# kouyt5/lightning-asr

Hardware: AMD Instinct MI355X
Metric: audio-seconds/sec training (asr13x1, bs=32, 10 s clips) (higher is better)
Workload: dtype bf16; 1 GPU; asr13x1 QuartzNet-CTC train step, bs=32/GPU, 10 s synthetic 16 kHz clips, labels.txt vocab (C=28), HIP mel+conv+CTC+NovoGrad, random-init weights; global_batch=32, n_class=28, parallelism=dp1, feature_prefetch=True, hip_graph=True, staged_backward=False

## Files before the change

lightning_asr_amd/csrc/fused.h:

```cpp
#pragma once
#include "common.h"

namespace lasr {

int dwconv_fwd_bn(const void* y, const float* coef, const void* y2, const float* coef2, int act, const float* w, void* out, void* u,
                  int64_t B, int64_t T, int64_t C, int k, void* stream);

static constexpr int kDwTapRow = 160;
struct DwTapJobs {
  int n; int blk0[17]; const float* w[16]; uint32_t* out[16]; int C[16]; int k[16];
};
__device__ __forceinline__ uint32_t dw_tap_entry(const float* __restrict__ w, int C, int k, int e) {
  const int flip = e / (C * kDwTapRow), r = e - flip * (C * kDwTapRow);
  const int c = r / kDwTapRow, idx = r - c * kDwTapRow;
  const int i0 = idx < kDwTapRow / 2 ? 2 * idx : 2 * (idx - kDwTapRow / 2) + 1;
  const int j0 = i0 - 24, j1 = i0 - 23;
  const float* wc = w + (size_t)c * k;
  const int q0 = min(max(j0, 0), k - 1), q1 = min(max(j1, 0), k - 1);
  const float a0 = wc[flip ? k - 1 - q0 : q0], a1 = wc[flip ? k - 1 - q1 : q1];
  const uint32_t m0 = (j0 >= 0 && j0 < k) ? 0xffffffffu : 0u, m1 = (j1 >= 0 && j1 < k) ? 0xffffffffu : 0u;
  return (uint32_t)f32_to_bf16(__uint_as_float(__float_as_uint(a0) & m0)) | ((uint32_t)f32_to_bf16(__uint_as_float(__float_as_uint(a1) & m1)) << 16);
}
struct DwTapCtx { int n; const float* w[16]; const uint32_t* t[16]; int C[16]; };
void dw_taps_set_ctx(const DwTapCtx* ctx);
const uint32_t* dw_taps_for(const float* w, int flip, int64_t C);
bool dw_taps_enabled();

int mask_lengths_step_cast(const float* pct, int64_t B, int64_t T_, int32_t* lens, uint64_t* step_counter, const float* in, void* out,
                           int64_t n, const DwTapJobs* jobs, void* stream);
int head_tail(const float* gl, int64_t rows, int64_t C, void* gl_bf16, int64_t ld_out, float* bias_grad, void* workspace,
              size_t workspace_bytes, const float* nll, int64_t n_nll, float scale, float* loss, void* stream);

int bn_se_act_fwd(const void* y, const float* coef, const void* y2, const float* coef2, const float* sums, const float* W1, const float* W2,
                  void* out, float* pooled, float* hidden, float* scale, int dtype, int64_t B, int64_t T_, int64_t C, int act, void* stream);

bool log_softmax_split_on(int64_t C);
int log_softmax_split(const float* partials, int split, const float* bias, float* logits, float* logp, int32_t* argmax, int64_t N, int64_t C,
                      void* stream);

}
```

lightning_asr_amd/csrc/model.hip:

```cpp
#include "common.h"
#include "mel.h"
#include "fused.h"
#include "gemm.h"
#include "lstm_body.h"
#include "se_seqsum.h"
#include <string>
#include <vector>
#include <math.h>

extern "C" size_t lasr_bn_bwd_workspace_bytes(int64_t B, int64_t T, int64_t C);
extern "C" size_t lasr_gemm_workspace_bytes(int64_t M, int64_t N, int split_k, int want_stats);
extern "C" size_t lasr_dwconv_wgrad_workspace_bytes(int64_t B, int64_t Tout, int64_t C, int k);
extern "C" int lasr_log_softmax_bwd(const float*, const float*, float*, int64_t, int64_t, void*);
extern "C" int lasr_cast_f32_to_bf16(const float*, void*, int64_t, void*);
extern "C" int lasr_colsum_f32(const float* x, float* out, int64_t rows, int64_t C, void* workspace, size_t workspace_bytes, void* stream);
extern "C" size_t lasr_colsum_workspace_bytes(int64_t rows, int64_t C);
extern "C" int lasr_scale_sum_f32(const float* x, int64_t n, float scale, float* out, void* stream);
extern "C" int lasr_seqsum(const void* x, int dtype, int64_t B, int64_t T, int64_t C, float* sums, void* stream);
extern "C" int lasr_se_fwd(const float* sums, const float* coef, const float* W1, const float* W2, int64_t B, int64_t T, int64_t C,
                           float* pooled, float* hidden, float* scale, void* stream);
extern "C" size_t lasr_se_bwd_workspace_bytes(int64_t B, int64_t C);
extern "C" int lasr_se_bwd(const void* dout, const void* y, const float* coef, const void* y2, const float* coef2, const float* scale,
                           const float* hidden, const float* pooled, const float* W1, const float* W2, int dtype, int64_t B, int64_t T,
                           int64_t C, int act, float* seg, float* dW1, float* dW2, void* workspace, size_t workspace_bytes, void* stream);
// ... 60 lines not shown
  size_t o_wgp = 0, wgp_bytes = 0, o_dwp = 0, dwp_bytes = 0, o_dy = 0, o_dy2 = 0;
  size_t o_taps = 0;
};

struct LstmRef { int64_t w_ih[2] = {-1, -1}, w_hh[2] = {-1, -1}, b_ih[2] = {-1, -1}, b_hh[2] = {-1, -1}; };

struct Plan {
  int64_t B = 0, T_in = 0, T = 0, S_max = 0;
  size_t total = 0;
  size_t o_lens = 0, o_logits = 0, o_glogits = 0, o_nll = 0, o_scratch = 0, o_g[2] = {0, 0}, o_d1 = 0, o_d2 = 0, o_du = 0, o_dxr = 0;
  size_t o_sums = 0, o_sums2 = 0, o_ctc = 0, o_wbf16 = 0;
  size_t o_cat = 0, o_gx[2] = {0, 0}, o_lstm_saved = 0, o_dg[2] = {0, 0};
  size_t o_dgb[2] = {0, 0}, o_lstm_part = 0, o_lstm_bpart = 0, o_lstm_wgp = 0, lstm_wgp_bytes = 0;
  size_t scratch_bytes = 0, ctc_bytes = 0;
  size_t o_rowstat = 0, o_lean = 0, lean_bytes = 0;
};

}

using namespace lasr;

struct lasr_model {
  lasr_model_config cfg;
  std::vector<TensorInfo> tensors;
  std::vector<Unit> units;
  int64_t n_param = 0, n_buffer = 0;
  int64_t w_dec = -1, b_dec = -1;
  LstmRef lstm;
  Plan plan;
  bool planned = false;
  float drop_p = 0.f;
  uint64_t drop_seed = 0;
  uint64_t* drop_step = nullptr;
  const float* tail_nll = nullptr; float* tail_loss = nullptr;
  bool lean_active = false;
  int lean_tiles = 0;
  int bwd_cur = 0;
  bool taps_valid = false;
  int bwd_next = -1;
  struct Prefetch {
    bool armed = false;
    WaveSrc src; const int32_t* sample_lens; const int32_t* aug;
    int64_t B, L; int normalize; void* out_btf; int dtype; int32_t* frames_out; float* pct_out; void* ws; size_t ws_bytes;
  } prefetch;

  int64_t add_tensor(const std::string& name, std::initializer_list<int64_t> shape, int kind) {
    TensorInfo t;
    t.name = name;
    t.kind = kind;
    t.ndim = (int)shape.size();
    int i = 0;
    for (int64_t s : shape) { t.shape[i++] = s; t.numel *= s; }
    if (kind == 0) { t.offset = n_param; n_param += t.numel; }
    else if (kind == 1) { t.offset = n_buffer; n_buffer += t.numel; }
// ... 172 lines not shown
  p.o_g[1] = take(cur, (size_t)N * cmax * es);
  p.o_d1 = take(cur, (size_t)N * std::max<int64_t>(cmax, (C + 7) / 8 * 8) * es);
  p.o_d2 = take(cur, (size_t)N * cmax * es);
  p.o_du = take(cur, (size_t)N * cmax * es);
  p.o_dxr = take(cur, (size_t)N * cmax * es);
  p.o_sums = take(cur, 2 * cmax * sizeof(float));
  p.o_sums2 = take(cur, 2 * cmax * sizeof(float));
  p.ctc_bytes = lasr_ctc_workspace_bytes(B, p.T, S_max);
  p.o_ctc = take(cur, p.ctc_bytes);
  if (lean_capable(m)) {
    p.o_rowstat = take(cur, lasr_gemm_rowstat_bytes(N, C));
    p.lean_bytes = lasr_ctc_lean_workspace_bytes(B, p.T, C, S_max);
    p.o_lean = take(cur, p.lean_bytes);
  }
  if (m->cfg.dtype == LASR_BF16) p.o_wbf16 = take(cur, (size_t)m->n_param * sizeof(bf16_t));
  p.total = cur;
  m->planned = true;
}

extern "C" int lasr_model_create(const lasr_model_config* cfg, lasr_model_t** out) {
  LASR_CHECK_ARG(cfg && out, "lasr_model_create: null pointer");
  LASR_CHECK_ARG(cfg->variant >= 0 && cfg->variant <= 2 && cfg->n_class >= 2 && cfg->in_c > 0 && cfg->in_c % 4 == 0,
                 "lasr_model_create: bad config (variant=%d n_class=%d in_c=%d)", cfg->variant, cfg->n_class, cfg->in_c);
  LASR_CHECK_ARG(cfg->dtype == LASR_F32 || cfg->dtype == LASR_BF16, "lasr_model_create: bad dtype");
  LASR_CHECK_ARG(cfg->act == LASR_ACT_RELU || cfg->act == LASR_ACT_SWISH, "lasr_model_create: bad activation");
  lasr_model* m = new lasr_model();
  m->cfg = *cfg;
  int rc = build_model(m);
  if (rc) { delete m; return rc; }
  *out = m;
// ... 76 lines not shown
    if (n == u.tap + ".y") { shape[0] = B; shape[1] = p.T; shape[2] = u.co; return (int64_t)u.o_y; }
    if (n == u.tap + ".y2" && u.has_res) { shape[0] = B; shape[1] = p.T; shape[2] = u.co; return (int64_t)u.o_y2; }
    if (n == u.tap + ".u" && u.has_dw) { shape[0] = B; shape[1] = p.T; shape[2] = u.ci; return (int64_t)u.o_u; }
    if (n == u.tap + ".se_hidden" && u.has_se) { shape[0] = B; shape[1] = 1; shape[2] = u.co / 8; return (int64_t)u.o_se_hid; }
  }
  if (n == "bwd.g_cur" || n == "bwd.g_prev") {
    int64_t cmax = 0;
    for (const Unit& u : m->units) cmax = std::max<int64_t>(cmax, std::max(u.ci, u.co));
    shape[0] = B; shape[1] = p.T; shape[2] = cmax;
    return (int64_t)p.o_g[n == "bwd.g_cur" ? m->bwd_cur : (m->bwd_cur ^ 1)];
  }
  if (n == "ctx_in" && m->cfg.variant != LASR_VARIANT_PLAIN) { shape[0] = B; shape[1] = p.T; shape[2] = 336; return (int64_t)p.o_cat; }
  if (n == "logits") { shape[0] = B; shape[1] = p.T; shape[2] = m->cfg.n_class; return (int64_t)p.o_logits; }
  if (n == "grad_logits") { shape[0] = B; shape[1] = p.T; shape[2] = m->cfg.n_class; return (int64_t)p.o_glogits; }
  if (n == "lens") { shape[0] = B; shape[1] = 1; shape[2] = 1; return (int64_t)p.o_lens; }
  if (n == "logits_bf16" && lean_capable(m)) { shape[0] = B; shape[1] = p.T; shape[2] = lean_ldc(m); return (int64_t)p.o_logits; }
  if (n == "grad_logits_bf16" && lean_capable(m)) { shape[0] = B; shape[1] = p.T; shape[2] = lean_ldc(m); return (int64_t)p.o_d1; }
  if (n == "lse" && lean_capable(m)) {
    shape[0] = B; shape[1] = p.T; shape[2] = 1;
    return (int64_t)(p.o_lean + align_up(lasr_ctc_workspace_bytes(B, p.T, p.S_max), 256));
  }
  return -1;
}

struct ProfScope {
  int tok; hipStream_t st;
  ProfScope(int kind, void* stream, double bytes) : tok(prof_begin(kind, as_stream(stream), 0.0, bytes)), st(as_stream(stream)) {}
  ~ProfScope() { prof_end(tok, st); }
};

// ... 56 lines not shown
    ProfScope ps(LASR_PROF_OTHER, stream, dt == LASR_BF16 ? 6.0 * m->n_param : 0.0);
    int merged = 1;
    m->taps_valid = false;
    if (dt == LASR_BF16) {
      DwTapJobs jobs;
      jobs.n = 0; jobs.blk0[0] = 0;
      {
        for (const Unit& u : m->units)
          if (u.o_taps && jobs.n < 16) {
            jobs.w[jobs.n] = params + u.w_dw; jobs.out[jobs.n] = reinterpret_cast<uint32_t*>(at(ws, u.o_taps)); jobs.C[jobs.n] = u.ci; jobs.k[jobs.n] = u.k;
            jobs.blk0[jobs.n + 1] = jobs.blk0[jobs.n] + (int)cdiv((int64_t)2 * u.ci * kDwTapRow, 256);
            ++jobs.n;
          }
      }
      merged = mask_lengths_step_cast(pct, B, T, lens, dropping ? m->drop_step : nullptr, params, at(ws, p.o_wbf16), m->n_param,
                                      jobs.n ? &jobs : nullptr, stream);
      if (merged < 0 || merged > 1) return merged;
      m->taps_valid = merged == 0 && jobs.n > 0;
    }
    if (merged == 1) {
      LASR_TRY(lasr_mask_lengths_step(pct, B, T, lens, dropping ? m->drop_step : nullptr, stream));
      if (dt == LASR_BF16) LASR_TRY(lasr_cast_f32_to_bf16(params, at(ws, p.o_wbf16), m->n_param, stream));
    }
  }
  DwTapScope tap_scope(m, params, ws, m->taps_valid);
  void* scratch = at(ws, p.o_scratch);
  if (!training) {
    std::vector<lasr_bn_eval_desc> descs;
    for (const Unit& u : m->units) {
      descs.push_back({params + u.bn.gamma, params + u.bn.beta, buffers + u.bn.rmean, buffers + u.bn.rvar, atf(ws, u.o_coef), u.co});
      if (u.has_res)
        descs.push_back({params + u.bn_res.gamma, params + u.bn_res.beta, buffers + u.bn_res.rmean, buffers + u.bn_res.rvar,
                         atf(ws, u.o_coef2), u.co});
    }
    for (size_t i = 0; i < descs.size(); i += 64)
      LASR_TRY(lasr_bn_eval_coef_many(descs.data() + i, (int)std::min<size_t>(64, descs.size() - i), kBnEps, stream));
    if (eval_fold(m->cfg.dtype)) {
      std::vector<lasr_fold_desc> fd;
      for (const Unit& u : m->units)
// ... 159 lines not shown
static int dec_wgrad_split(int64_t C, int64_t N) {
  const int64_t tiles = cdiv(C, 128) * 8;
  const double t_k = 15.8e-9;
  const double t_slab = (double)C * 1024 * 8 / 4e12;
  int best = 1;
  double best_t = 1e30;
  for (int sp = 1; sp <= 16; ++sp) {
    const double rounds = (double)cdiv(tiles * sp, 512);
    const double t = rounds * (double)cdiv(N, sp) * t_k + (sp > 1 ? sp * t_slab : 0.0);
    if (t < best_t) { best_t = t; best = sp; }
  }
  return best;
}

static int backward_from_glogits(lasr_model* m, const float* params, const void* feats, int64_t B, int64_t T_in, float* grads,
                                 void* ws, void* stream, bool with_head = true, int unit_hi = -1, int unit_stop = 0) {
  const Plan& p = m->plan;
  const int dt = m->cfg.dtype;
  const int64_t T = p.T, N = B * T, C = m->cfg.n_class;
  DwTapScope tap_scope(m, params, ws, m->taps_valid);
  void* scratch = at(ws, p.o_scratch);
  const size_t sb = p.scratch_bytes;
  const int32_t* lens = reinterpret_cast<const int32_t*>(at(ws, p.o_lens));
  float* gl = atf(ws, p.o_glogits);
  const Unit& last = m->units.back();
  int cur = m->bwd_cur;
  const float* tail_nll = m->tail_nll;
  float* tail_loss = m->tail_loss;
  m->tail_nll = nullptr; m->tail_loss = nullptr;
  if (with_head) {
  cur = 0;
// ... 60 lines not shown
      LASR_TRY(lasr_bn_se_bwd(dout, at(ws, u.o_y), atf(ws, u.o_coef), atf(ws, u.o_saved), params + u.bn.gamma, params + u.bn.beta,
                              u.has_res ? at(ws, u.o_y2) : nullptr, u.has_res ? atf(ws, u.o_coef2) : nullptr,
                              u.has_res ? atf(ws, u.o_saved2) : nullptr, u.has_res ? params + u.bn_res.gamma : nullptr, se_scale,
                              atf(ws, u.o_se_hid), atf(ws, u.o_se_pool), atf(ws, u.o_se_sum), params + u.w_se1, params + u.w_se2,
                              u.masked ? lens : nullptr, dy, dy2, grads + u.bn.gamma, grads + u.bn.beta,
                              u.has_res ? grads + u.bn_res.gamma : nullptr, u.has_res ? grads + u.bn_res.beta : nullptr, grads + u.w_se1,
                              grads + u.w_se2, atf(ws, u.o_se_grad), dt, B, T, u.co, act, dq, scratch, sb, stream));
    } else {
    if (u.has_se)
      LASR_TRY(lasr_se_bwd_drop(dout, at(ws, u.o_y), atf(ws, u.o_coef), u.has_res ? at(ws, u.o_y2) : nullptr,
                                u.has_res ? atf(ws, u.o_coef2) : nullptr, se_scale, atf(ws, u.o_se_hid), atf(ws, u.o_se_pool), params + u.w_se1,
                                params + u.w_se2, dt, B, T, u.co, act, dq, atf(ws, u.o_se_grad), grads + u.w_se1, grads + u.w_se2, scratch, sb,
                                stream));
    float* fsum = no_fuse() ? atf(ws, p.o_sums) : nullptr;
    float* fsum2 = no_fuse() ? atf(ws, p.o_sums2) : nullptr;
    LASR_TRY(lasr_bn_act_bwd_stats_drop(dout, at(ws, u.o_y), atf(ws, u.o_coef), atf(ws, u.o_saved), u.has_res ? at(ws, u.o_y2) : nullptr,
                                        u.has_res ? atf(ws, u.o_coef2) : nullptr, u.has_res ? atf(ws, u.o_saved2) : nullptr, se_scale,
                                        se_grad, fsum, fsum2, dt, B, T, u.co, act, dq, scratch, sb, stream));
    LASR_TRY(lasr_bn_act_bwd_apply_drop(dout, at(ws, u.o_y), atf(ws, u.o_coef), atf(ws, u.o_saved), params + u.bn.gamma,
                                        u.has_res ? at(ws, u.o_y2) : nullptr, u.has_res ? atf(ws, u.o_coef2) : nullptr,
                                        u.has_res ? atf(ws, u.o_saved2) : nullptr, u.has_res ? params + u.bn_res.gamma : nullptr, se_scale,
                                        se_grad, fsum, fsum2, u.masked ? lens : nullptr, dy, dy2,
                                        grads + u.bn.gamma, grads + u.bn.beta, u.has_res ? grads + u.bn_res.gamma : nullptr,
                                        u.has_res ? grads + u.bn_res.beta : nullptr, dt, B, T, u.co, act, dq, scratch, sb, stream));
    }
    }
    const void* gin = u.has_dw ? at(ws, u.o_u) : x_in;
    {
      lasr_gemm_problem pr[2];
      pr[0] = {dy, gin, grads + u.w_pw, u.co, u.ci, N, nullptr, nullptr, 0, nullptr};
      if (u.has_res) pr[1] = {dy2, x_in, grads + u.w_res, u.co, u.ci, N, nullptr, nullptr, 0, nullptr};
      if (defer_w) {
        float* slab = atf(ws, u.o_wgp);
        if (wprobs.size() + (u.has_res ? 2 : 1) > 32) LASR_TRY(flush_wgrads(wprobs, wslabs, pending, stream));
        wprobs.push_back(pr[0]); wslabs.push_back(slab);
        if (u.has_res) { wprobs.push_back(pr[1]); wslabs.push_back(slab + u.wgp_bytes / (2 * sizeof(float))); }
      } else {
        LASR_TRY(lasr_gemm_batch(pr, u.has_res ? 2 : 1, dt, LASR_F32, 1, 1, wgrad_split(), scratch, sb, stream));
      }
// ... 178 lines not shown

extern "C" int lasr_model_unit_info(const lasr_model_t* m, int64_t i, char* name, size_t name_cap) {
  LASR_CHECK_ARG(m && i >= 0 && i < (int64_t)m->units.size() && name && name_cap > 0, "lasr_model_unit_info: bad argument");
  strncpy(name, m->units[i].tap.c_str(), name_cap - 1);
  name[name_cap - 1] = 0;
  return 0;
}

extern "C" int lasr_model_loss_backward_partial(lasr_model_t* m, const float* params, float* buffers, const void* feats, const float* pct,
                                                const int64_t* targets, const int32_t* tgt_lens, int64_t B, int64_t T_in, int64_t S_max,
                                                float* logp_out, float* loss_out, float* nll_out, int32_t* argmax_out, float* grads,
                                                void* ws, size_t ws_bytes, int64_t unit_stop, void* stream) {
  LASR_CHECK_ARG(m && unit_stop >= 0 && unit_stop < (int64_t)m->units.size(), "lasr_model_loss_backward_partial: unit_stop");
  LASR_TRY(forward_and_loss(m, params, buffers, feats, pct, targets, tgt_lens, B, T_in, S_max, logp_out, loss_out, nll_out, argmax_out, grads,
                            ws, ws_bytes, stream, "lasr_model_loss_backward_partial"));
  return backward_from_glogits(m, params, feats, B, T_in, grads, ws, stream, true, -1, (int)unit_stop);
}

extern "C" int lasr_model_backward_continue(lasr_model_t* m, const float* params, const void* feats, int64_t B, int64_t T_in, float* grads,
                                            void* ws, size_t ws_bytes, int64_t unit_stop, void* stream) {
  LASR_CHECK_ARG(m && params && feats && grads && ws, "lasr_model_backward_continue: null pointer");
  LASR_CHECK_ARG(m->planned && m->plan.B == B && m->plan.T_in == T_in && m->bwd_next >= 0, "lasr_model_backward_continue: nothing pending");
  LASR_CHECK_ARG(unit_stop >= 0 && unit_stop <= m->bwd_next, "lasr_model_backward_continue: unit_stop");
  if (ws_bytes < m->plan.total) return fail(LASR_E_WORKSPACE, "lasr_model_backward_continue: workspace");
  return backward_from_glogits(m, params, feats, B, T_in, grads, ws, stream, false, m->bwd_next, (int)unit_stop);
}
```

lightning_asr_amd/csrc/norm.hip:

```cpp
#include "common.h"
#include "reduce_body.h"
#include "se_seqsum.h"
#include "fused.h"
#include "dropout.h"
#include <algorithm>
#include <string.h>

namespace lasr {

template <typename T, bool TO_BTC>
__global__ __launch_bounds__(256) void transpose_kernel(const void* __restrict__ in_, void* __restrict__ out_,
                                                        int64_t C, int64_t Tt) {
  __shared__ float tile[32][33];
  const int b = blockIdx.z;
  const int64_t c0 = (int64_t)blockIdx.y * 32, t0 = (int64_t)blockIdx.x * 32;
  const int tx = threadIdx.x & 31, ty = threadIdx.x >> 5;
  if (TO_BTC) {
    const float* in = reinterpret_cast<const float*>(in_) + (int64_t)b * C * Tt;
    T* out = reinterpret_cast<T*>(out_) + (int64_t)b * C * Tt;
    for (int i = ty; i < 32; i += 8)
      if (c0 + i < C && t0 + tx < Tt) tile[i][tx] = in[(c0 + i) * Tt + t0 + tx];
    __syncthreads();
    for (int i = ty; i < 32; i += 8)
      if (t0 + i < Tt && c0 + tx < C) Elem<T>::st(out + (t0 + i) * C + c0 + tx, tile[tx][i]);
  } else {
    const T* in = reinterpret_cast<const T*>(in_) + (int64_t)b * C * Tt;
    float* out = reinterpret_cast<float*>(out_) + (int64_t)b * C * Tt;
    for (int i = ty; i < 32; i += 8)
      if (t0 + i < Tt && c0 + tx < C) tile[i][tx] = Elem<T>::ld(in + (t0 + i) * C + c0 + tx);
    __syncthreads();
    for (int i = ty; i < 32; i += 8)
      if (c0 + i < C && t0 + tx < Tt) out[(c0 + i) * Tt + t0 + tx] = tile[tx][i];
  }
}

__global__ void mask_lengths_kernel(const float* __restrict__ pct, int64_t B, float Tf, int32_t* __restrict__ lens,
                                    unsigned long long* __restrict__ step_counter) {
  const int64_t i = blockIdx.x * (int64_t)blockDim.x + threadIdx.x;
  if (i < B) lens[i] = (int32_t)(Tf * pct[i]);
  if (i == 0 && step_counter) *step_counter += 1ull;
}

__global__ __launch_bounds__(256) void mask_lengths_cast_kernel(const float* __restrict__ pct, int64_t B, float Tf, int32_t* __restrict__ lens,
                                                                unsigned long long* __restrict__ step_counter, const float* __restrict__ in,
                                                                bf16_t* __restrict__ out, int64_t n, int cast_blocks, DwTapJobs jobs) {
  if (blockIdx.x == gridDim.x - 1) {
    for (int64_t i = threadIdx.x; i < B; i += 256) lens[i] = (int32_t)(Tf * pct[i]);
    if (threadIdx.x == 0 && step_counter) *step_counter += 1ull;
    return;
  }
  if ((int)blockIdx.x >= cast_blocks) {
    const int tb = (int)blockIdx.x - cast_blocks;
    int l = 0;
    while (l + 1 < jobs.n && jobs.blk0[l + 1] <= tb) ++l;
    const int e = (tb - jobs.blk0[l]) * 256 + (int)threadIdx.x;
    if (e < 2 * jobs.C[l] * kDwTapRow) jobs.out[l][e] = dw_tap_entry(jobs.w[l], jobs.C[l], jobs.k[l], e);
    return;
  }
  const int64_t n4 = n >> 2;
  const int64_t stride = (int64_t)cast_blocks * 256;
  for (int64_t e = blockIdx.x * (int64_t)256 + threadIdx.x; e < n4; e += stride) {
    const float4 v = reinterpret_cast<const float4*>(in)[e];
// ... 703 lines not shown
        if (live) Vec<bf16_t>::store(dy2 + off[u], o2);
      }
    }
  }
  });
}

static int bn_sliced_rpc(int dtype, int64_t rows, int64_t C, bool se, bool drop, int per_utt, bool reduced_sums) {
  static const int target = getenv("LASR_BN_SLICED") ? atoi(getenv("LASR_BN_SLICED")) : 256;
  if (target <= 0 || dtype != LASR_BF16 || se || drop || per_utt || reduced_sums || C % kSlCh != 0 || rows < 4096) return 0;
  const int64_t slices = C / kSlCh;
  const int64_t nchunk = std::max<int64_t>(1, std::min<int64_t>(target / slices, rows / kSlLanes));
  return (int)cdiv(rows, nchunk);
}

}

using namespace lasr;

extern "C" int lasr_bn_act_bwd_stats_drop(const void* dout, const void* y, const float* coef, const float* saved, const void* y2,
                                          const float* coef2, const float* saved2, const float* se_scale, const float* se_grad,
                                          float* sums, float* sums2, int dtype, int64_t B, int64_t T_, int64_t C, int act,
                                          const lasr_dropout* dropout, void* workspace, size_t workspace_bytes, void* stream);
extern "C" int lasr_bn_act_bwd_apply_drop(const void* dout, const void* y, const float* coef, const float* saved,
                                          const float* gamma, const void* y2, const float* coef2, const float* saved2,
                                          const float* gamma2, const float* se_scale, const float* se_grad, const float* sums,
                                          const float* sums2, const int32_t* row_lens, void* dy, void* dy2, float* dgamma,
                                          float* dbeta, float* dgamma2, float* dbeta2, int dtype, int64_t B, int64_t T_, int64_t C,
                                          int act, const lasr_dropout* dropout, void* workspace, size_t workspace_bytes, void* stream);

// ... 24 lines not shown
  LASR_CHECK_SHAPE(B > 0 && C > 0 && T_ > 0 && B < 65536, "lasr_bct_to_btc: shape");
  dim3 grid((unsigned)cdiv(T_, 32), (unsigned)cdiv(C, 32), (unsigned)B);
  DISPATCH_DTYPE(dtype, hipLaunchKernelGGL((transpose_kernel<T, true>), grid, dim3(256), 0, as_stream(stream), in, out, C, T_));
  LASR_LAUNCH_CHECK("transpose_kernel");
  return 0;
}
extern "C" int lasr_btc_to_bct(const void* in, int dtype, float* out, int64_t B, int64_t C, int64_t T_, void* stream) {
  LASR_CHECK_ARG(in && out && (dtype == LASR_F32 || dtype == LASR_BF16), "lasr_btc_to_bct: bad argument");
  LASR_CHECK_SHAPE(B > 0 && C > 0 && T_ > 0 && B < 65536, "lasr_btc_to_bct: shape");
  dim3 grid((unsigned)cdiv(T_, 32), (unsigned)cdiv(C, 32), (unsigned)B);
  DISPATCH_DTYPE(dtype, hipLaunchKernelGGL((transpose_kernel<T, false>), grid, dim3(256), 0, as_stream(stream), in, out, C, T_));
  LASR_LAUNCH_CHECK("transpose_kernel");
  return 0;
}

extern "C" int lasr_mask_lengths_step(const float* pct, int64_t B, int64_t T_, int32_t* lens, uint64_t* step_counter, void* stream) {
  LASR_CHECK_ARG(pct && lens && B > 0 && T_ > 0, "lasr_mask_lengths: bad argument");
  hipLaunchKernelGGL(mask_lengths_kernel, dim3((unsigned)cdiv(B, 256)), dim3(256), 0, as_stream(stream), pct, B, (float)T_, lens,
                     reinterpret_cast<unsigned long long*>(step_counter));
  LASR_LAUNCH_CHECK("mask_lengths_kernel");
  return 0;
}
int lasr::mask_lengths_step_cast(const float* pct, int64_t B, int64_t T_, int32_t* lens, uint64_t* step_counter, const float* in, void* out,
                                 int64_t n, const DwTapJobs* jobs, void* stream) {
  LASR_CHECK_ARG(pct && lens && B > 0 && T_ > 0 && in && out && n > 0, "mask_lengths_step_cast: bad argument");
  if (reinterpret_cast<uintptr_t>(in) % 16 || reinterpret_cast<uintptr_t>(out) % 8) return 1;
  int64_t blocks = cdiv(n >> 2, 256);
  if (blocks > 256 * 8) blocks = 256 * 8;
  if (blocks < 1) blocks = 1;
  DwTapJobs j;
  memset(&j, 0, sizeof(j));
  int tap_blocks = 0;
  if (jobs) {
    j = *jobs;
    tap_blocks = j.blk0[j.n];
  }
  hipLaunchKernelGGL(mask_lengths_cast_kernel, dim3((unsigned)(blocks + tap_blocks + 1)), dim3(256), 0, as_stream(stream), pct, B, (float)T_, lens,
                     reinterpret_cast<unsigned long long*>(step_counter), in, reinterpret_cast<bf16_t*>(out), n, (int)blocks, j);
  LASR_LAUNCH_CHECK("mask_lengths_cast_kernel");
  return 0;
}

extern "C" int lasr_mask_lengths(const float* pct, int64_t B, int64_t T_, int32_t* lens, void* stream) {
  return lasr_mask_lengths_step(pct, B, T_, lens, nullptr, stream);
}

namespace lasr {
__global__ __launch_bounds__(256) void dropout_mask_kernel(DropArgs d, int64_t n, uint8_t* __restrict__ keep) {
  const int64_t v = (int64_t)blockIdx.x * 256 + threadIdx.x;
  if (v * 8 >= n) return;
  const uint32_t m = d.step ? drop_keep8(d, *d.step, (uint32_t)v) : 0xffu;
  for (int i = 0; i < 8 && v * 8 + i < n; ++i) keep[v * 8 + i] = (m >> i) & 1u;
}
// ... 140 lines not shown
                                             partials, (int)rows, (int)T_, (int)C, act, da, per_utt); } }); }
  } else {
    if (se_scale) { DISPATCH_DTYPE(dtype, { if (da.step) { hipLaunchKernelGGL((bn_bwd_stats_kernel<T, false, true, true>), dim3(nblk), dim3(256), shmem, as_stream(stream),
                                             (const T*)dout, (const T*)y, coef, saved, (const T*)y2, coef2, saved2, se_scale, se_grad,
                                             partials, (int)rows, (int)T_, (int)C, act, da, per_utt); } else { hipLaunchKernelGGL((bn_bwd_stats_kernel<T, false, true, false>), dim3(nblk), dim3(256), shmem, as_stream(stream),
                                             (const T*)dout, (const T*)y, coef, saved, (const T*)y2, coef2, saved2, se_scale, se_grad,
                                             partials, (int)rows, (int)T_, (int)C, act, da, per_utt); } }); } else { DISPATCH_DTYPE(dtype, { if (da.step) { hipLaunchKernelGGL((bn_bwd_stats_kernel<T, false, false, true>), dim3(nblk), dim3(256), shmem, as_stream(stream),
                                             (const T*)dout, (const T*)y, coef, saved, (const T*)y2, coef2, saved2, se_scale, se_grad,
                                             partials, (int)rows, (int)T_, (int)C, act, da, per_utt); } else { hipLaunchKernelGGL((bn_bwd_stats_kernel<T, false, false, false>), dim3(nblk), dim3(256), shmem, as_stream(stream),
                                             (const T*)dout, (const T*)y, coef, saved, (const T*)y2, coef2, saved2, se_scale, se_grad,
                                             partials, (int)rows, (int)T_, (int)C, act, da, per_utt); } }); }
  }
  LASR_LAUNCH_CHECK("bn_bwd_stats_kernel");
  if (!sums) return 0;
  return launch_reduce_partials(partials, nblk, 4 * C, sums, 2 * C, sums2, as_stream(stream));
}

extern "C" size_t lasr_bn_bwd_apply_workspace_bytes(int64_t C) { return (size_t)10 * C * sizeof(float); }

extern "C" int lasr_bn_act_bwd_apply(const void* dout, const void* y, const float* coef, const float* saved,
                                     const float* gamma, const void* y2, const float* coef2, const float* saved2,
                                     const float* gamma2, const float* se_scale, const float* se_grad, const float* sums,
                                     const float* sums2, const int32_t* row_lens, void* dy, void* dy2, float* dgamma,
                                     float* dbeta, float* dgamma2, float* dbeta2, int dtype, int64_t B, int64_t T_, int64_t C,
                                     int act, void* workspace, size_t workspace_bytes, void* stream) {
  return lasr_bn_act_bwd_apply_drop(dout, y, coef, saved, gamma, y2, coef2, saved2, gamma2, se_scale, se_grad, sums, sums2, row_lens, dy, dy2,
                                    dgamma, dbeta, dgamma2, dbeta2, dtype, B, T_, C, act, nullptr, workspace, workspace_bytes, stream);
}

extern "C" int lasr_bn_act_bwd_apply_drop(const void* dout, const void* y, const float* coef, const float* saved,
// ... 357 lines not shown
```

Baseline: 160,100 audio-seconds/sec.

## Fuse BN-activation backward stats and apply into one persistent grid-synced kernel

Adds a one-pass batchnorm+activation backward kernel. Each workgroup keeps its rows of dout/y in registers, publishes per-channel partial sums, waits on an agent-scope arrival counter (with work-stealing and a timeout fallback), then applies the gradient without re-reading inputs. It replaces the separate stats, reduce and apply launches for non-SE bf16 units, cutting launches and a second full pass over activations. In exchange it adds inter-workgroup spin synchronization that needs all workgroups co-resident, sync words zeroed each step inside the mask-lengths kernel, and a per-unit fallback when the kernel declines or times out.

```diff
diff --git a/lightning_asr_amd/csrc/fused.h b/lightning_asr_amd/csrc/fused.h
--- a/lightning_asr_amd/csrc/fused.h
+++ b/lightning_asr_amd/csrc/fused.h
@@ -27,7 +27,9 @@
 bool dw_taps_enabled();
 
 int mask_lengths_step_cast(const float* pct, int64_t B, int64_t T_, int32_t* lens, uint64_t* step_counter, const float* in, void* out,
-                           int64_t n, const DwTapJobs* jobs, void* stream);
+                           int64_t n, const DwTapJobs* jobs, uint32_t* zero, int nzero, void* stream);
+int mask_lengths_step_zero(const float* pct, int64_t B, int64_t T_, int32_t* lens, uint64_t* step_counter, uint32_t* zero, int nzero,
+                           void* stream);
 int head_tail(const float* gl, int64_t rows, int64_t C, void* gl_bf16, int64_t ld_out, float* bias_grad, void* workspace,
               size_t workspace_bytes, const float* nll, int64_t n_nll, float scale, float* loss, void* stream);
 
@@ -38,4 +40,13 @@
 int log_softmax_split(const float* partials, int split, const float* bias, float* logits, float* logp, int32_t* argmax, int64_t N, int64_t C,
                       void* stream);
 
+static constexpr int kBnOnepassMaxSlices = 32;
+static constexpr int kBnOnepassSyncWords = 2 * kBnOnepassMaxSlices;
+
 }
+
+extern "C" int lasr_bn_act_bwd_onepass(const void* dout, const void* y, const float* coef, const float* saved, const float* gamma,
+                                       const void* y2, const float* coef2, const float* saved2, const float* gamma2,
+                                       const int32_t* row_lens, void* dy, void* dy2, float* dgamma, float* dbeta, float* dgamma2,
+                                       float* dbeta2, int dtype, int64_t B, int64_t T_, int64_t C, int act, void* workspace,
+                                       size_t workspace_bytes, uint32_t* status, uint32_t* sync, void* stream);
diff --git a/lightning_asr_amd/csrc/model.hip b/lightning_asr_amd/csrc/model.hip
--- a/lightning_asr_amd/csrc/model.hip
+++ b/lightning_asr_amd/csrc/model.hip
@@ -98,6 +98,7 @@
   size_t o_dgb[2] = {0, 0}, o_lstm_part = 0, o_lstm_bpart = 0, o_lstm_wgp = 0, lstm_wgp_bytes = 0;
   size_t scratch_bytes = 0, ctc_bytes = 0;
   size_t o_rowstat = 0, o_lean = 0, lean_bytes = 0;
+  size_t o_bnsync = 0, bnsync_words = 0;
 };
 
 }
@@ -122,6 +123,7 @@
   int bwd_cur = 0;
   bool taps_valid = false;
   int bwd_next = -1;
+  std::vector<char> bnsync_armed;
   struct Prefetch {
     bool armed = false;
     WaveSrc src; const int32_t* sample_lens; const int32_t* aug;
@@ -324,6 +326,8 @@
     p.o_lean = take(cur, p.lean_bytes);
   }
   if (m->cfg.dtype == LASR_BF16) p.o_wbf16 = take(cur, (size_t)m->n_param * sizeof(bf16_t));
+  p.bnsync_words = 2 + m->units.size() * (size_t)kBnOnepassSyncWords;
+  p.o_bnsync = take(cur, p.bnsync_words * sizeof(uint32_t));
   p.total = cur;
   m->planned = true;
 }
@@ -430,6 +434,10 @@
   if (n == "logits") { shape[0] = B; shape[1] = p.T; shape[2] = m->cfg.n_class; return (int64_t)p.o_logits; }
   if (n == "grad_logits") { shape[0] = B; shape[1] = p.T; shape[2] = m->cfg.n_class; return (int64_t)p.o_glogits; }
   if (n == "lens") { shape[0] = B; shape[1] = 1; shape[2] = 1; return (int64_t)p.o_lens; }
+  if (n == "bn_onepass.err" || n == "bn_onepass.stolen") {
+    shape[0] = 1; shape[1] = 1; shape[2] = 1;
+    return (int64_t)(p.o_bnsync + (n == "bn_onepass.err" ? 0 : sizeof(uint32_t)));
+  }
   if (n == "logits_bf16" && lean_capable(m)) { shape[0] = B; shape[1] = p.T; shape[2] = lean_ldc(m); return (int64_t)p.o_logits; }
   if (n == "grad_logits_bf16" && lean_capable(m)) { shape[0] = B; shape[1] = p.T; shape[2] = lean_ldc(m); return (int64_t)p.o_d1; }
   if (n == "lse" && lean_capable(m)) {
@@ -516,15 +524,17 @@
           }
       }
       merged = mask_lengths_step_cast(pct, B, T, lens, dropping ? m->drop_step : nullptr, params, at(ws, p.o_wbf16), m->n_param,
-                                      jobs.n ? &jobs : nullptr, stream);
+                                      jobs.n ? &jobs : nullptr, reinterpret_cast<uint32_t*>(at(ws, p.o_bnsync)), (int)p.bnsync_words, stream);
       if (merged < 0 || merged > 1) return merged;
       m->taps_valid = merged == 0 && jobs.n > 0;
     }
     if (merged == 1) {
-      LASR_TRY(lasr_mask_lengths_step(pct, B, T, lens, dropping ? m->drop_step : nullptr, stream));
+      LASR_TRY(mask_lengths_step_zero(pct, B, T, lens, dropping ? m->drop_step : nullptr, reinterpret_cast<uint32_t*>(at(ws, p.o_bnsync)),
+                                      (int)p.bnsync_words, stream));
       if (dt == LASR_BF16) LASR_TRY(lasr_cast_f32_to_bf16(params, at(ws, p.o_wbf16), m->n_param, stream));
     }
   }
+  m->bnsync_armed.assign(m->units.size(), 1);
   DwTapScope tap_scope(m, params, ws, m->taps_valid);
   void* scratch = at(ws, p.o_scratch);
   if (!training) {
@@ -714,7 +724,8 @@
 }
 
 static int backward_from_glogits(lasr_model* m, const float* params, const void* feats, int64_t B, int64_t T_in, float* grads,
-                                 void* ws, void* stream, bool with_head = true, int unit_hi = -1, int unit_stop = 0) {
+                                 void* ws, void* stream, bool with_head = true, int unit_hi = -1, int unit_stop = 0,
+                                 bool staged = false) {
   const Plan& p = m->plan;
   const int dt = m->cfg.dtype;
   const int64_t T = p.T, N = B * T, C = m->cfg.n_class;
@@ -805,6 +816,19 @@
                                 stream));
     float* fsum = no_fuse() ? atf(ws, p.o_sums) : nullptr;
     float* fsum2 = no_fuse() ? atf(ws, p.o_sums2) : nullptr;
+    int onepass = 1;
+    if (!staged && !no_fuse() && !u.has_se && !dq && dt == LASR_BF16 && (size_t)ui < m->bnsync_armed.size() && m->bnsync_armed[ui]) {
+      uint32_t* words = reinterpret_cast<uint32_t*>(at(ws, p.o_bnsync));
+      onepass = lasr_bn_act_bwd_onepass(dout, at(ws, u.o_y), atf(ws, u.o_coef), atf(ws, u.o_saved), params + u.bn.gamma,
+                                        u.has_res ? at(ws, u.o_y2) : nullptr, u.has_res ? atf(ws, u.o_coef2) : nullptr,
+                                        u.has_res ? atf(ws, u.o_saved2) : nullptr, u.has_res ? params + u.bn_res.gamma : nullptr,
+                                        u.masked ? lens : nullptr, dy, dy2, grads + u.bn.gamma, grads + u.bn.beta,
+                                        u.has_res ? grads + u.bn_res.gamma : nullptr, u.has_res ? grads + u.bn_res.beta : nullptr, dt, B, T,
+                                        u.co, act, scratch, sb, words, words + 2 + (size_t)ui * kBnOnepassSyncWords, stream);
+      if (onepass < 0) return onepass;
+      if (onepass == 0) m->bnsync_armed[ui] = 0;
+    }
+    if (onepass == 1) {
     LASR_TRY(lasr_bn_act_bwd_stats_drop(dout, at(ws, u.o_y), atf(ws, u.o_coef), atf(ws, u.o_saved), u.has_res ? at(ws, u.o_y2) : nullptr,
                                         u.has_res ? atf(ws, u.o_coef2) : nullptr, u.has_res ? atf(ws, u.o_saved2) : nullptr, se_scale,
                                         se_grad, fsum, fsum2, dt, B, T, u.co, act, dq, scratch, sb, stream));
@@ -814,6 +838,7 @@
                                         se_grad, fsum, fsum2, u.masked ? lens : nullptr, dy, dy2,
                                         grads + u.bn.gamma, grads + u.bn.beta, u.has_res ? grads + u.bn_res.gamma : nullptr,
                                         u.has_res ? grads + u.bn_res.beta : nullptr, dt, B, T, u.co, act, dq, scratch, sb, stream));
+    }
     }
     }
     const void* gin = u.has_dw ? at(ws, u.o_u) : x_in;
@@ -1022,7 +1047,7 @@
   LASR_CHECK_ARG(m && unit_stop >= 0 && unit_stop < (int64_t)m->units.size(), "lasr_model_loss_backward_partial: unit_stop");
   LASR_TRY(forward_and_loss(m, params, buffers, feats, pct, targets, tgt_lens, B, T_in, S_max, logp_out, loss_out, nll_out, argmax_out, grads,
                             ws, ws_bytes, stream, "lasr_model_loss_backward_partial"));
-  return backward_from_glogits(m, params, feats, B, T_in, grads, ws, stream, true, -1, (int)unit_stop);
+  return backward_from_glogits(m, params, feats, B, T_in, grads, ws, stream, true, -1, (int)unit_stop, true);
 }
 
 extern "C" int lasr_model_backward_continue(lasr_model_t* m, const float* params, const void* feats, int64_t B, int64_t T_in, float* grads,
@@ -1031,5 +1056,5 @@
   LASR_CHECK_ARG(m->planned && m->plan.B == B && m->plan.T_in == T_in && m->bwd_next >= 0, "lasr_model_backward_continue: nothing pending");
   LASR_CHECK_ARG(unit_stop >= 0 && unit_stop <= m->bwd_next, "lasr_model_backward_continue: unit_stop");
   if (ws_bytes < m->plan.total) return fail(LASR_E_WORKSPACE, "lasr_model_backward_continue: workspace");
-  return backward_from_glogits(m, params, feats, B, T_in, grads, ws, stream, false, m->bwd_next, (int)unit_stop);
-}
+  return backward_from_glogits(m, params, feats, B, T_in, grads, ws, stream, false, m->bwd_next, (int)unit_stop, true);
+}
diff --git a/lightning_asr_amd/csrc/norm.hip b/lightning_asr_amd/csrc/norm.hip
--- a/lightning_asr_amd/csrc/norm.hip
+++ b/lightning_asr_amd/csrc/norm.hip
@@ -35,17 +35,21 @@
 }
 
 __global__ void mask_lengths_kernel(const float* __restrict__ pct, int64_t B, float Tf, int32_t* __restrict__ lens,
-                                    unsigned long long* __restrict__ step_counter) {
+                                    unsigned long long* __restrict__ step_counter, uint32_t* __restrict__ zero, int nzero) {
   const int64_t i = blockIdx.x * (int64_t)blockDim.x + threadIdx.x;
   if (i < B) lens[i] = (int32_t)(Tf * pct[i]);
+  if (blockIdx.x == 0)
+    for (int e = threadIdx.x; e < nzero; e += blockDim.x) zero[e] = 0u;
   if (i == 0 && step_counter) *step_counter += 1ull;
 }
 
 __global__ __launch_bounds__(256) void mask_lengths_cast_kernel(const float* __restrict__ pct, int64_t B, float Tf, int32_t* __restrict__ lens,
                                                                 unsigned long long* __restrict__ step_counter, const float* __restrict__ in,
-                                                                bf16_t* __restrict__ out, int64_t n, int cast_blocks, DwTapJobs jobs) {
+                                                                bf16_t* __restrict__ out, int64_t n, int cast_blocks, DwTapJobs jobs,
+                                                                uint32_t* __restrict__ zero, int nzero) {
   if (blockIdx.x == gridDim.x - 1) {
     for (int64_t i = threadIdx.x; i < B; i += 256) lens[i] = (int32_t)(Tf * pct[i]);
+    for (int e = threadIdx.x; e < nzero; e += 256) zero[e] = 0u;
     if (threadIdx.x == 0 && step_counter) *step_counter += 1ull;
     return;
   }
@@ -779,6 +783,312 @@
   return (int)cdiv(rows, nchunk);
 }
 
+static constexpr int kOpMaxSteal = 256;
+static constexpr uint32_t kOpErrTimeout = 1u;
+
+struct OnepassLds {
+  float red[8][4][kSlCh];
+  double sum[4][kSlCh];
+  __attribute__((aligned(16))) float tab[10][kSlCh];
+  __attribute__((aligned(16))) float mq[4][kSlCh];
+  int stolen[kOpMaxSteal];
+  int ctl[4];
+};
+
+template <bool HAS2>
+__device__ __forceinline__ void onepass_stats_row(const OnepassLds& s, int cl, const uint4& rd, const uint4& ry, const uint4& rr, float live,
+                                                  bool lead, int act, float (&acc)[4][8]) {
+  constexpr int V = 8;
+  __atomic_signal_fence(__ATOMIC_SEQ_CST);
+  float dvi[V], yvi[V], rvi[V], d[V];
+  Vec<bf16_t>::unpack(rd, dvi);
+  Vec<bf16_t>::unpack(ry, yvi);
+  if (HAS2) Vec<bf16_t>::unpack(rr, rvi);
+  {
+    float a1[V], b1[V], a2[V], b2[V];
+    lds_vec8(&s.tab[0][cl * V], a1); lds_vec8(&s.tab[1][cl * V], b1);
+    if (HAS2) { lds_vec8(&s.tab[5][cl * V], a2); lds_vec8(&s.tab[6][cl * V], b2); }
+#pragma unroll
+    for (int j = 0; j < V; ++j) {
+      const float z = fmaf(yvi[j], a1[j], b1[j]) * 1.f + (HAS2 ? fmaf(rvi[j], a2[j], b2[j]) : 0.f);
+      const float g = act_grad(z, act);
+      d[j] = dvi[j] * g * live;
+      if (!HAS2 && lead) acc[0][j] = live != 0.f ? fmaf(dvi[j], g, acc[0][j]) : acc[0][j];
+    }
+  }
+  {
+    float m1[V], q1[V];
+    lds_vec8(&s.mq[0][cl * V], m1); lds_vec8(&s.mq[1][cl * V], q1);
+#pragma unroll
+    for (int j = 0; j < V; ++j) {
+      if (HAS2 || !lead) acc[0][j] += d[j];
+      acc[1][j] = fmaf(d[j], (yvi[j] - m1[j]) * q1[j], acc[1][j]);
+    }
+  }
+  if (HAS2) {
+    float m2[V], q2[V];
+    lds_vec8(&s.mq[2][cl * V], m2); lds_vec8(&s.mq[3][cl * V], q2);
+#pragma unroll
+    for (int j = 0; j < V; ++j) {
+      acc[2][j] += d[j];
+      acc[3][j] = fmaf(d[j], (rvi[j] - m2[j]) * q2[j], acc[3][j]);
+    }
+  }
+}
+
+__device__ __forceinline__ void onepass_publish(OnepassLds& s, float (&acc)[4][8], float* prow, int C, uint32_t* arrive) {
+  constexpr int V = 8;
+  const int tid = threadIdx.x, cl = tid & 7, lane = tid & 63, wid = tid >> 6;
+#pragma unroll
+  for (int k = 0; k < 4; ++k)
+#pragma unroll
+    for (int j = 0; j < V; ++j) {
+      float v = acc[k][j];
+      v += __shfl_xor(v, 8, 64); v += __shfl_xor(v, 16, 64); v += __shfl_xor(v, 32, 64);
+      acc[k][j] = v;
+    }
+  if (lane < 8) {
+#pragma unroll
+    for (int k = 0; k < 4; ++k)
+#pragma unroll
+      for (int j = 0; j < V; ++j) s.red[wid][k][cl * V + j] = acc[k][j];
+  }
+  __syncthreads();
+  if (tid < 4 * kSlCh) {
+    const int k = tid >> 6, ch = tid & 63;
+    float t = 0.f;
+#pragma unroll
+    for (int w = 0; w < 8; ++w) t += s.red[w][k][ch];
+    __hip_atomic_store(prow + (size_t)k * C + ch, t, __ATOMIC_RELAXED, __HIP_MEMORY_SCOPE_AGENT);
+  }
+  __syncthreads();
+  if (tid == 0) {
+    __builtin_amdgcn_fence(__ATOMIC_RELEASE, "agent");
+    __hip_atomic_fetch_add(arrive, 1u, __ATOMIC_RELAXED, __HIP_MEMORY_SCOPE_AGENT);
+  }
+}
+
+template <bool HAS2, int act>
+__device__ __forceinline__ void onepass_apply_row(const OnepassLds& s, int cl, const uint4& rd, const uint4& ry, const uint4& rr2, bool masked,
+                                                  bool live, bf16_t* __restrict__ dy, bf16_t* __restrict__ dy2, uint32_t off) {
+  constexpr int V = 8;
+  float dv[V], yv[V], rv[V], o1[V], o2[V];
+  Vec<bf16_t>::unpack(rd, dv);
+  Vec<bf16_t>::unpack(ry, yv);
+  if (HAS2) Vec<bf16_t>::unpack(rr2, rv);
+  float ca[V], cb[V], G[V], Bc[V], Cc[V], z[V], d[V];
+  lds_vec8(&s.tab[0][cl * V], ca); lds_vec8(&s.tab[1][cl * V], cb);
+#pragma unroll
+  for (int j = 0; j < V; ++j) z[j] = fmaf(yv[j], ca[j], cb[j]) * 1.f;
+  if (HAS2) {
+    lds_vec8(&s.tab[5][cl * V], ca); lds_vec8(&s.tab[6][cl * V], cb);
+#pragma unroll
+    for (int j = 0; j < V; ++j) z[j] += fmaf(rv[j], ca[j], cb[j]);
+  }
+#pragma unroll
+  for (int j = 0; j < V; ++j) d[j] = dv[j] * act_grad(z[j], act);
+  lds_vec8(&s.tab[2][cl * V], G); lds_vec8(&s.tab[3][cl * V], Bc); lds_vec8(&s.tab[4][cl * V], Cc);
+#pragma unroll
+  for (int j = 0; j < V; ++j) o1[j] = masked ? 0.f : fmaf(G[j], d[j], fmaf(Bc[j], yv[j], Cc[j]));
+  if (live) Vec<bf16_t>::store(dy + off, o1);
+  if (HAS2) {
+    lds_vec8(&s.tab[7][cl * V], G); lds_vec8(&s.tab[8][cl * V], Bc); lds_vec8(&s.tab[9][cl * V], Cc);
+#pragma unroll
+    for (int j = 0; j < V; ++j) o2[j] = fmaf(G[j], d[j], fmaf(Bc[j], rv[j], Cc[j]));
+    if (live) Vec<bf16_t>::store(dy2 + off, o2);
+  }
+}
+
+template <bool HAS2, int RPT>
+__global__ __launch_bounds__(512) void bn_bwd_onepass_sliced_kernel(const bf16_t* __restrict__ dout, const bf16_t* __restrict__ y,
+                                                                    const bf16_t* __restrict__ y2, float* partials, int nchunk,
+                                                                    const float* __restrict__ coef, const float* __restrict__ saved,
+                                                                    const float* __restrict__ gamma, const float* __restrict__ coef2,
+                                                                    const float* __restrict__ saved2, const float* __restrict__ gamma2,
+                                                                    float inv_n, const int32_t* __restrict__ row_lens, bf16_t* __restrict__ dy,
+                                                                    bf16_t* __restrict__ dy2, float* __restrict__ dgamma, float* __restrict__ dbeta,
+                                                                    float* __restrict__ dgamma2, float* __restrict__ dbeta2, int rows, int Tt,
+                                                                    int C, int act_rt, int rpc, uint32_t* status, uint32_t* sync,
+                                                                    unsigned patience, unsigned cap) {
+  __shared__ OnepassLds s;
+  constexpr int V = 8;
+  const int tid = threadIdx.x, cl = tid & 7, rl = tid >> 3;
+  const int c0 = blockIdx.x * kSlCh, c = c0 + cl * V;
+  uint32_t* ticket = sync + 2 * blockIdx.x;
+  uint32_t* arrive = ticket + 1;
+  if (tid == 0) {
+    s.ctl[1] = (int)__hip_atomic_fetch_add(ticket, 1u, __ATOMIC_RELAXED, __HIP_MEMORY_SCOPE_AGENT);
+    s.ctl[2] = 0;
+  }
+  if (tid < kSlCh) {
+    const int ch = c0 + tid;
+    s.tab[0][tid] = coef[ch]; s.tab[1][tid] = coef[C + ch]; s.mq[0][tid] = saved[ch]; s.mq[1][tid] = saved[C + ch];
+    if (HAS2) { s.tab[5][tid] = coef2[ch]; s.tab[6][tid] = coef2[C + ch]; s.mq[2][tid] = saved2[ch]; s.mq[3][tid] = saved2[C + ch]; }
+    else { s.tab[5][tid] = s.tab[6][tid] = s.mq[2][tid] = s.mq[3][tid] = 0.f; }
+  }
+  __syncthreads();
+  const int chunk = s.ctl[1];
+  if (chunk >= nchunk) return;
+  const int r0 = chunk * rpc, r1 = min(r0 + rpc, rows);
+  const int nk = (r1 - r0 + kSlLanes - 1) / kSlLanes;
+  uint4 rd[RPT], ry[RPT], rr[RPT];
+#pragma unroll
+  for (int k = 0; k < RPT; ++k) {
+    if (k < nk) {
+      const uint32_t off = (uint32_t)min(r0 + rl + k * kSlLanes, rows - 1) * (uint32_t)C + (uint32_t)c;
+      rd[k] = Vec<bf16_t>::raw(dout + off);
+      ry[k] = Vec<bf16_t>::raw(y + off);
+      if (HAS2) rr[k] = Vec<bf16_t>::raw(y2 + off);
+    }
+  }
+  {
+    const int act = act_rt;
+    float acc[4][V];
+#pragma unroll
+    for (int k = 0; k < 4; ++k)
+#pragma unroll
+      for (int j = 0; j < V; ++j) acc[k][j] = 0.f;
+#pragma unroll
+    for (int k = 0; k < RPT; ++k) {
+      if (k < nk) onepass_stats_row<HAS2>(s, cl, rd[k], ry[k], rr[k], r0 + rl + k * kSlLanes < r1 ? 1.f : 0.f, (k & 3) == 0, act, acc);
+    }
+    onepass_publish(s, acc, partials + (size_t)chunk * 4 * C + c0, C, arrive);
+  }
+  for (;;) {
+    if (tid == 0) {
+      const unsigned long long t0 = wall_clock64();
+      bool dealt = false;
+      int state = 0;
+      for (;;) {
+        if (__hip_atomic_load(arrive, __ATOMIC_RELAXED, __HIP_MEMORY_SCOPE_AGENT) >= (uint32_t)nchunk) break;
+        const unsigned long long el = wall_clock64() - t0;
+        if (!dealt && (s.ctl[2] > 0 || el >= patience)) {
+          dealt = __hip_atomic_load(ticket, __ATOMIC_RELAXED, __HIP_MEMORY_SCOPE_AGENT) >= (uint32_t)nchunk;
+          if (!dealt) {
+            const uint32_t t = __hip_atomic_fetch_add(ticket, 1u, __ATOMIC_RELAXED, __HIP_MEMORY_SCOPE_AGENT);
+            if (t < (uint32_t)nchunk) { s.ctl[1] = (int)t; state = 1; break; }
+            dealt = true;
+          }
+        }
+        if (el > cap) { state = 2; break; }
+        __builtin_amdgcn_s_sleep(16);
+      }
+      if (state == 0) __builtin_amdgcn_fence(__ATOMIC_ACQUIRE, "agent");
+      if (state == 1) {
+        if (s.ctl[2] < kOpMaxSteal) s.stolen[s.ctl[2]] = s.ctl[1];
+        s.ctl[2] += 1;
+        __hip_atomic_fetch_add(status + 1, 1u, __ATOMIC_RELAXED, __HIP_MEMORY_SCOPE_AGENT);
+      }
+      if (state == 2) __hip_atomic_fetch_or(status, kOpErrTimeout, __ATOMIC_RELAXED, __HIP_MEMORY_SCOPE_AGENT);
+      s.ctl[0] = state;
+    }
+    __syncthreads();
+    const int state = s.ctl[0];
+    if (state == 2) return;
+    if (state == 0) break;
+    const int taken = s.ctl[1];
+    const int q0 = taken * rpc, q1 = min(q0 + rpc, rows);
+    const int act = act_rt;
+    float acc[4][V];
+#pragma unroll
+    for (int k = 0; k < 4; ++k)
+#pragma unroll
+      for (int j = 0; j < V; ++j) acc[k][j] = 0.f;
+    for (int rb = q0 + rl, m = 0; rb < q1; rb += 2 * kSlLanes, ++m) {
+      uint4 sd[2], sy[2], sr[2];
+#pragma unroll
+      for (int i = 0; i < 2; ++i) {
+        const uint32_t off = (uint32_t)min(rb + i * kSlLanes, rows - 1) * (uint32_t)C + (uint32_t)c;
+        sd[i] = Vec<bf16_t>::raw(dout + off);
+        sy[i] = Vec<bf16_t>::raw(y + off);
+        if (HAS2) sr[i] = Vec<bf16_t>::raw(y2 + off);
+      }
+#pragma unroll
+      for (int i = 0; i < 2; ++i)
+        onepass_stats_row<HAS2>(s, cl, sd[i], sy[i], sr[i], rb + i * kSlLanes < q1 ? 1.f : 0.f, i == 0 && (m & 1) == 0, act, acc);
+    }
+    onepass_publish(s, acc, partials + (size_t)taken * 4 * C + c0, C, arrive);
+    __syncthreads();
+  }
+  if (tid < 4 * kSlCh) {
+    const int k = tid >> 6, ch = tid & 63;
+    double a0 = 0.0, a1 = 0.0;
+    if (k < 2 || HAS2) {
+      float* p = partials + (size_t)k * C + c0 + ch;
+      for (int q = 0; q < nchunk; q += 16) {
+        float v[16];
+#pragma unroll
+        for (int i = 0; i < 16; ++i) {
+          const float x = __hip_atomic_load(p + (size_t)min(q + i, nchunk - 1) * 4 * C, __ATOMIC_RELAXED, __HIP_MEMORY_SCOPE_AGENT);
+          v[i] = q + i < nchunk ? x : 0.f;
+        }
+#pragma unroll
+        for (int i = 0; i < 16; i += 2) { a0 += (double)v[i]; a1 += (double)v[i + 1]; }
+      }
+    }
+    s.sum[k][ch] = a0 + a1;
+  }
+  __syncthreads();
+  if (tid < kSlCh) {
+    bool has0 = chunk == 0;
+    for (int i = 0; i < min(s.ctl[2], kOpMaxSteal); ++i) has0 = has0 || s.stolen[i] == 0;
+    const int ch = c0 + tid;
+    const float s1 = (float)s.sum[0][tid], s2 = (float)s.sum[1][tid];
+    {
+      const float q = saved[C + ch], w = s2 * inv_n, G = gamma[ch] * q;
+      s.tab[2][tid] = G; s.tab[3][tid] = -G * q * w;
+      s.tab[4][tid] = G * (saved[ch] * q * w - s1 * inv_n);
+      if (has0) { dbeta[ch] = s1; dgamma[ch] = s2; }
+    }
+    if (HAS2) {
+      const float s1b = (float)s.sum[2][tid], s2b = (float)s.sum[3][tid];
+      const float q = saved2[C + ch], w = s2b * inv_n, G = gamma2[ch] * q;
+      s.tab[7][tid] = G; s.tab[8][tid] = -G * q * w;
+      s.tab[9][tid] = G * (saved2[ch] * q * w - s1b * inv_n);
+      if (has0) { dbeta2[ch] = s1b; dgamma2[ch] = s2b; }
+    } else {
+      s.tab[7][tid] = s.tab[8][tid] = s.tab[9][tid] = 0.f;
+    }
+  }
+  __syncthreads();
+  with_act(act_rt, [&](auto act_c) {
+    constexpr int act = decltype(act_c)::value;
+#pragma unroll
+    for (int k = 0; k < RPT; ++k) {
+      if (k < nk) {
+        const int r = r0 + rl + k * kSlLanes;
+        const int rc = min(r, rows - 1);
+        const int ub = rc / Tt;
+        const bool masked = row_lens && (rc - ub * Tt) >= row_lens[ub];
+        onepass_apply_row<HAS2, act>(s, cl, rd[k], ry[k], rr[k], masked, r < r1, dy, dy2, (uint32_t)rc * (uint32_t)C + (uint32_t)c);
+      }
+    }
+    const int ns = min(s.ctl[2], kOpMaxSteal);
+    for (int i = 0; i < ns; ++i) {
+      const int q0 = s.stolen[i] * rpc, q1 = min(q0 + rpc, rows);
+      for (int rb = q0 + rl; rb < q1; rb += 2 * kSlLanes) {
+        uint4 sd[2], sy[2], sr[2];
+        uint32_t off[2];
+#pragma unroll
+        for (int u = 0; u < 2; ++u) {
+          off[u] = (uint32_t)min(rb + u * kSlLanes, rows - 1) * (uint32_t)C + (uint32_t)c;
+          sd[u] = Vec<bf16_t>::raw(dout + off[u]);
+          sy[u] = Vec<bf16_t>::raw(y + off[u]);
+          if (HAS2) sr[u] = Vec<bf16_t>::raw(y2 + off[u]);
+        }
+#pragma unroll
+        for (int u = 0; u < 2; ++u) {
+          const int r = rb + u * kSlLanes;
+          const int rc = min(r, rows - 1);
+          const int ub = rc / Tt;
+          const bool masked = row_lens && (rc - ub * Tt) >= row_lens[ub];
+          onepass_apply_row<HAS2, act>(s, cl, sd[u], sy[u], sr[u], masked, r < q1, dy, dy2, off[u]);
+        }
+      }
+    }
+  });
+}
+
 }
 
 using namespace lasr;
@@ -833,15 +1143,19 @@
   return 0;
 }
 
-extern "C" int lasr_mask_lengths_step(const float* pct, int64_t B, int64_t T_, int32_t* lens, uint64_t* step_counter, void* stream) {
-  LASR_CHECK_ARG(pct && lens && B > 0 && T_ > 0, "lasr_mask_lengths: bad argument");
+int lasr::mask_lengths_step_zero(const float* pct, int64_t B, int64_t T_, int32_t* lens, uint64_t* step_counter, uint32_t* zero, int nzero,
+                                 void* stream) {
+  LASR_CHECK_ARG(pct && lens && B > 0 && T_ > 0 && (zero || nzero == 0), "lasr_mask_lengths: bad argument");
   hipLaunchKernelGGL(mask_lengths_kernel, dim3((unsigned)cdiv(B, 256)), dim3(256), 0, as_stream(stream), pct, B, (float)T_, lens,
-                     reinterpret_cast<unsigned long long*>(step_counter));
+                     reinterpret_cast<unsigned long long*>(step_counter), zero, nzero);
   LASR_LAUNCH_CHECK("mask_lengths_kernel");
   return 0;
 }
+extern "C" int lasr_mask_lengths_step(const float* pct, int64_t B, int64_t T_, int32_t* lens, uint64_t* step_counter, void* stream) {
+  return lasr::mask_lengths_step_zero(pct, B, T_, lens, step_counter, nullptr, 0, stream);
+}
 int lasr::mask_lengths_step_cast(const float* pct, int64_t B, int64_t T_, int32_t* lens, uint64_t* step_counter, const float* in, void* out,
-                                 int64_t n, const DwTapJobs* jobs, void* stream) {
+                                 int64_t n, const DwTapJobs* jobs, uint32_t* zero, int nzero, void* stream) {
   LASR_CHECK_ARG(pct && lens && B > 0 && T_ > 0 && in && out && n > 0, "mask_lengths_step_cast: bad argument");
   if (reinterpret_cast<uintptr_t>(in) % 16 || reinterpret_cast<uintptr_t>(out) % 8) return 1;
   int64_t blocks = cdiv(n >> 2, 256);
@@ -855,7 +1169,7 @@
     tap_blocks = j.blk0[j.n];
   }
   hipLaunchKernelGGL(mask_lengths_cast_kernel, dim3((unsigned)(blocks + tap_blocks + 1)), dim3(256), 0, as_stream(stream), pct, B, (float)T_, lens,
-                     reinterpret_cast<unsigned long long*>(step_counter), in, reinterpret_cast<bf16_t*>(out), n, (int)blocks, j);
+                     reinterpret_cast<unsigned long long*>(step_counter), in, reinterpret_cast<bf16_t*>(out), n, (int)blocks, j, zero, nzero);
   LASR_LAUNCH_CHECK("mask_lengths_cast_kernel");
   return 0;
 }
@@ -1026,6 +1340,58 @@
   LASR_LAUNCH_CHECK("bn_bwd_stats_kernel");
   if (!sums) return 0;
   return launch_reduce_partials(partials, nblk, 4 * C, sums, 2 * C, sums2, as_stream(stream));
+}
+
+extern "C" int lasr_bn_act_bwd_onepass(const void* dout, const void* y, const float* coef, const float* saved, const float* gamma,
+                                       const void* y2, const float* coef2, const float* saved2, const float* gamma2,
+                                       const int32_t* row_lens, void* dy, void* dy2, float* dgamma, float* dbeta, float* dgamma2,
+                                       float* dbeta2, int dtype, int64_t B, int64_t T_, int64_t C, int act, void* workspace,
+                                       size_t workspace_bytes, uint32_t* status, uint32_t* sync, void* stream) {
+  static const bool on = !getenv("LASR_BN_ONEPASS") || atoi(getenv("LASR_BN_ONEPASS")) > 0;
+  static const int wgs_env = getenv("LASR_BN_ONEPASS_WGS") ? atoi(getenv("LASR_BN_ONEPASS_WGS")) : 0;
+  if (!on || (nt_loads_mask() & 3)) return 1;
+  LASR_CHECK_ARG(dout && y && coef && saved && gamma && dy && dgamma && dbeta && workspace && status && sync,
+                 "lasr_bn_act_bwd_onepass: null pointer");
+  LASR_CHECK_ARG(!y2 || (coef2 && saved2 && gamma2 && dy2 && dgamma2 && dbeta2), "lasr_bn_act_bwd_onepass: branch-2 pointers");
+  LASR_TRY(check_bn_shape("lasr_bn_act_bwd_onepass", dtype, B, T_, C));
+  const int64_t rows = B * T_;
+  const int rpc = bn_sliced_rpc(dtype, rows, C, false, false, 0, false);
+  if (!rpc) return 1;
+  const int slices = (int)(C / kSlCh), nchunk = (int)cdiv(rows, rpc), nk = (int)cdiv(rpc, kSlLanes);
+  if (slices > kBnOnepassMaxSlices || nchunk > kOpMaxSteal || nk > (y2 ? 8 : 16)) return 1;
+  struct DevInfo { int cus; int occ[2][3]; };
+  static DevInfo info[16];
+  static bool have[16];
+  int dev = 0;
+  if (hipGetDevice(&dev) != hipSuccess || dev < 0 || dev >= 16) return 1;
+  if (!have[dev]) {
+    DevInfo d;
+    if (hipDeviceGetAttribute(&d.cus, hipDeviceAttributeMultiprocessorCount, dev) != hipSuccess) return 1;
+#define LASR_OP_OCC(H2_, I_, R_)                                                                                                     \
+  if (hipOccupancyMaxActiveBlocksPerMultiprocessor(&d.occ[H2_][I_], bn_bwd_onepass_sliced_kernel<(H2_) != 0, R_>, kSlThreads, 0) != \
+      hipSuccess)                                                                                                                    \
+    d.occ[H2_][I_] = 0
+    LASR_OP_OCC(0, 0, 4); LASR_OP_OCC(0, 1, 8); LASR_OP_OCC(0, 2, 16);
+    LASR_OP_OCC(1, 0, 4); LASR_OP_OCC(1, 1, 8); d.occ[1][2] = 0;
+#undef LASR_OP_OCC
+    info[dev] = d; have[dev] = true;
+  }
+  const int ri = nk <= 4 ? 0 : nk <= 8 ? 1 : 2;
+  if (info[dev].cus < slices * nchunk || info[dev].occ[y2 ? 1 : 0][ri] < 1) return 1;
+  if (workspace_bytes < (size_t)nchunk * 4 * C * sizeof(float)) return fail(LASR_E_WORKSPACE, "lasr_bn_act_bwd_onepass: workspace");
+  const int wgs = wgs_env > 0 ? std::min(wgs_env, nchunk) : nchunk;
+  const dim3 grid((unsigned)slices, (unsigned)wgs);
+  const unsigned patience = 2000u, cap = 400000u;
+#define LASR_ONEPASS(H2_, R_)                                                                                                          \
+  hipLaunchKernelGGL((bn_bwd_onepass_sliced_kernel<H2_, R_>), grid, dim3(kSlThreads), 0, as_stream(stream), (const bf16_t*)dout,       \
+                     (const bf16_t*)y, (const bf16_t*)y2, reinterpret_cast<float*>(workspace), nchunk, coef, saved, gamma, coef2, saved2, \
+                     gamma2, 1.0f / (float)rows, row_lens, (bf16_t*)dy, (bf16_t*)dy2, dgamma, dbeta, dgamma2, dbeta2, (int)rows, (int)T_, \
+                     (int)C, act, rpc, status, sync, patience, cap)
+  if (y2) { if (ri == 0) LASR_ONEPASS(true, 4); else LASR_ONEPASS(true, 8); }
+  else { if (ri == 0) LASR_ONEPASS(false, 4); else if (ri == 1) LASR_ONEPASS(false, 8); else LASR_ONEPASS(false, 16); }
+#undef LASR_ONEPASS
+  LASR_LAUNCH_CHECK("bn_bwd_onepass_sliced_kernel");
+  return 0;
 }
 
 extern "C" size_t lasr_bn_bwd_apply_workspace_bytes(int64_t C) { return (size_t)10 * C * sizeof(float); }
```

Result: slower. 146,700 audio-seconds/sec (-8.4%).
